# lslrh/DynaMask

Measured on AMD Instinct MI355X. Metric: img/s (DynaMask mask-head path, 512 RoIs/img, fixed 28x28 exit; ms_per_step = ms per RoI batch), higher is better.
Workload: dtype f32

## Files before the change

dynamask_amd/csrc/conv_igemm.hip:

```cpp
#include <type_traits>

#include "common.h"

namespace {

struct ConvArgs {
  const float* src[DM_MAX_SOURCES];
  int src_c[DM_MAX_SOURCES];
  long long src_bs[DM_MAX_SOURCES];
  int num_srcs;
  int NB, H, W, HW, Q;
  const float* wq;
  const float* bias;
  int KQ, Cout, CoutP;
  int relu;
  float* out;
  int out_ch_total, out_ch_offset;
  int Wp, plane;
  int MT;
  int q_begin = 0;
  int shuffle;
  const float* mask = nullptr;
  int off32 = 0;
  float* ws = nullptr;
// ... 2 lines not shown
  int want_split = 0;
  const float* addend = nullptr;
};

typedef __bf16 dm_bf16x8 __attribute__((ext_vector_type(8)));

__device__ __forceinline__ void dm_split3(float x, __bf16& h, __bf16& m, __bf16& l) {
  h = (__bf16)x;
  const float hf = (float)h;
  if (__builtin_isfinite(hf)) {
    const float r1 = x - hf;
    m = (__bf16)r1;
    l = (__bf16)(r1 - (float)m);
  } else {
    m = (__bf16)0.f;
    l = (__bf16)0.f;
  }
}

__device__ __forceinline__ void dm_split8x3(const dm_f32x4& q0, const dm_f32x4& q1, dm_f32x4 (&out)[3]) {
  dm_bf16x8 w[3];
#pragma unroll
  for (int e = 0; e < 8; ++e) {
    __bf16 h, m, l;
    dm_split3(e < 4 ? q0[e] : q1[e - 4], h, m, l);
    w[0][e] = h;
    w[1][e] = m;
    w[2][e] = l;
  }
#pragma unroll
  for (int p = 0; p < 3; ++p) out[p] = __builtin_bit_cast(dm_f32x4, w[p]);
}

template <int KS, int WGM, int WGN, int WM, int WN, int CK, int MAXPOS, int TAIL = 0, int PREC = 0, int POST = 0>
__device__ __forceinline__ void conv_igemm_body(const ConvArgs& a, const int bx, const int gx, const int by) {
  static_assert(TAIL == 0 || (TAIL == 4 && WGM == 1), "tail rows need a single cout tile");
  static_assert(PREC == 0 || (PREC == 1 && CK == 16 && TAIL == 0 && WM == 1 && WN == 2 && WGM == 2 && WGN == 2),
                "the bf16x3 build: 64 x 128 tiles, 16-channel chunks, no tail rows");
  static_assert(POST == 0 || (KS == 1 && TAIL == 0 && PREC == 0), "the post-activation addend: exact fp32 1x1 builds");
  constexpr int TM = WGM * WM * 32;
  constexpr int TMA = TM + TAIL;
  constexpr int TN = WGN * WN * 32;
  constexpr int NT = WGM * WGN * 64;
  constexpr int TAPS = KS * KS;
  constexpr int NQ = CK / 4;
  constexpr int NWC = PREC ? 6 : NQ;
  constexpr int A_F4 = TAPS * NWC * TMA;
  constexpr int A_PER_T = (A_F4 + NT - 1) / NT;
  constexpr int B1_PER_T = (NQ * TN + NT - 1) / NT;
  constexpr int BREG = (KS == 3) ? MAXPOS * NQ : B1_PER_T;

  extern __shared__ __attribute__((aligned(16))) float lds[];
  dm_f32x4* ldsA = reinterpret_cast<dm_f32x4*>(lds);
  dm_f32x4* ldsB = reinterpret_cast<dm_f32x4*>(lds) + A_F4;

  const int tid = threadIdx.x;
  const int lane = tid & 63;
  const int wave = tid >> 6;
  const int wave_m = wave / WGN;
  const int wave_n = wave % WGN;
  const int hi = lane >> 5;
  const int l31 = lane & 31;

  int m_tile, n_tile;
  {
    const int b = bx, grp = 8 * a.MT;
    const int full = (gx / grp) * grp;
    if (b < full) {
      const int g = b / grp, r = b - g * grp;
      m_tile = r / 8;
      n_tile = g * 8 + (r & 7);
    } else {
      const int r = b - full;
      m_tile = r % a.MT;
      n_tile = full / a.MT + r / a.MT;
    }
  }
  const int m0 = m_tile * TM;
  const int q0 = a.q_begin + n_tile * TN;
  const int HW = a.HW, W = a.W, H = a.H;
  const int plane = a.plane;
  int k_skip = 0, k_left = 0x7fffffff;
  float* e_out = a.out;
  const float* e_bias = a.bias;
  const float* e_mask = a.mask;
  int e_relu = a.relu, e_oct = a.out_ch_total, e_oco = a.out_ch_offset;
  if (a.ksplit > 1) {
// ... 179 lines not shown
    } else if (KS == 3) {
#pragma unroll
      for (int k = 0; k < MAXPOS; ++k) {
        const bool ok = st_n[k] >= 0;
        const float* gp = sp + b_off[k];
#pragma unroll
        for (int qd = 0; qd < NQ; ++qd) {
          dm_f32x4 v = {0.f, 0.f, 0.f, 0.f};
#pragma unroll
          for (int e = 0; e < 4; ++e) {
            const int ci = qd * 4 + e;
            if (ok && ci < ckv) v[e] = gp[(size_t)ci * HW];
          }
          rb[k * NQ + qd] = v;
        }
      }
    } else {
      const bool ok = st_n[0] >= 0;
      const float* gp = sp + b_off[0];
#pragma unroll
      for (int i = 0; i < B1_PER_T; ++i) {
        const int qd = PREC ? (tid / TN) * 2 + i : tid / TN + i * (NT / TN);
        dm_f32x4 v = {0.f, 0.f, 0.f, 0.f};
#pragma unroll
        for (int e = 0; e < 4; ++e) {
          const int ci = qd * 4 + e;
          if (ok && qd < NQ && ci < ckv) v[e] = gp[(size_t)ci * HW];
        }
        rb[i] = v;
      }
    }
  };

  auto commit = [&]() {
#pragma unroll
    for (int i = 0; i < A_PER_T; ++i) {
      const int idx = tid + i * NT;
      if (idx < A_F4) ldsA[idx] = ra[i];
    }
    if (PREC) {
      if (KS == 3) {
#pragma unroll
        for (int k = 0; k < MAXPOS; ++k) {
          const int pos = tid + k * NT;
          if (pos < plane) {
#pragma unroll
            for (int h8 = 0; h8 < 2; ++h8) {
              dm_f32x4 wd[3];
              dm_split8x3(rb[k * NQ + 2 * h8], rb[k * NQ + 2 * h8 + 1], wd);
#pragma unroll
              for (int p_ = 0; p_ < 3; ++p_) ldsB[(3 * h8 + p_) * plane + pos] = wd[p_];
            }
          }
        }
      } else {
        static_assert(!PREC || KS == 3 || (B1_PER_T == 2 && NT / TN == 2), "1x1 bf16x3 build: two quads (one half) per thread");
        const int h8 = tid / TN;
        dm_f32x4 wd[3];
        dm_split8x3(rb[0], rb[B1_PER_T > 1 ? 1 : 0], wd);
#pragma unroll
        for (int p_ = 0; p_ < 3; ++p_) ldsB[(3 * h8 + p_) * plane + (tid % TN)] = wd[p_];
      }
    } else if (KS == 3) {
#pragma unroll
      for (int k = 0; k < MAXPOS; ++k) {
        const int pos = tid + k * NT;
        if (pos < plane) {
#pragma unroll
          for (int qd = 0; qd < NQ; ++qd) ldsB[qd * plane + pos] = rb[k * NQ + qd];
        }
      }
    } else {
#pragma unroll
      for (int i = 0; i < B1_PER_T; ++i) {
        const int qd = tid / TN + i * (NT / TN);
        if (qd < NQ) ldsB[qd * plane + (tid % TN)] = rb[i];
      }
    }
  };

  for (; k_skip > 0 && cs < a.num_srcs; --k_skip) chunk_advance();
  if (chunk_valid()) prefetch();
  while (chunk_valid()) {
    const int ckv_cur = min(CK, curC - cc0);
    const int ngroups = (ckv_cur + 7) / 8;
    commit();
    __syncthreads();
    chunk_advance();
    --k_left;
    if (chunk_valid()) prefetch();

    if (PREC) {
      auto load_frag = [&](int tap, dm_f32x4 (*av)[3], dm_f32x4 (*bv)[3]) {
        const int tapoff = (KS == 3) ? ((tap / 3) * Wp + (tap % 3)) : 0;
#pragma unroll
        for (int i = 0; i < WM; ++i)
#pragma unroll
          for (int p_ = 0; p_ < 3; ++p_) av[i][p_] = ldsA[(tap * NWC + 3 * hi + p_) * TMA + (wave_m * WM + i) * 32 + l31];
#pragma unroll
        for (int j = 0; j < WN; ++j)
#pragma unroll
          for (int p_ = 0; p_ < 3; ++p_) bv[j][p_] = ldsB[p_ * plane + lane_base[j] + tapoff];
      };
      auto mfma = [&](const dm_f32x4& x, const dm_f32x4& y, dm_f32x16& c) {
        c = __builtin_amdgcn_mfma_f32_32x32x16_bf16(__builtin_bit_cast(dm_bf16x8, x), __builtin_bit_cast(dm_bf16x8, y), c, 0, 0, 0);
      };
      dm_f32x4 av[2][WM][3], bv[2][WN][3];
      load_frag(0, av[0], bv[0]);
#pragma unroll
      for (int st = 0; st < TAPS; ++st) {
        const int cur = st & 1;
        if (st + 1 < TAPS) load_frag(st + 1, av[cur ^ 1], bv[cur ^ 1]);
#pragma unroll
        for (int i = 0; i < WM; ++i)
#pragma unroll
          for (int j = 0; j < WN; ++j) {
            mfma(av[cur][i][2], bv[cur][j][0], accx[i][j]);
            mfma(av[cur][i][1], bv[cur][j][1], accx[i][j]);
            mfma(av[cur][i][0], bv[cur][j][2], accx[i][j]);
            mfma(av[cur][i][1], bv[cur][j][0], accx[i][j]);
            mfma(av[cur][i][0], bv[cur][j][1], accx[i][j]);
            mfma(av[cur][i][0], bv[cur][j][0], acc[i][j]);
          }
      }
    } else {
      constexpr int NG = NQ / 2;
      constexpr int STEPS = TAPS * NG;
      auto load_frag = [&](int st, dm_f32x4* av, dm_f32x4* bv) {
        const int tap = st / NG, g = st - tap * NG;
        const int tapoff = (KS == 3) ? ((tap / 3) * Wp + (tap % 3)) : 0;
#pragma unroll
        for (int i = 0; i < WM; ++i) av[i] = ldsA[(tap * NQ + 2 * g + hi) * TMA + (wave_m * WM + i) * 32 + l31];
        if (TAIL) av[WM] = ldsA[(tap * NQ + 2 * g + hi) * TMA + TM + (lane & 3)];
#pragma unroll
        for (int j = 0; j < WN; ++j) bv[j] = ldsB[(2 * g) * plane + lane_base[j] + tapoff];
      };
      dm_f32x4 av[2][WM + (TAIL ? 1 : 0)], bv[2][WN];
      load_frag(0, av[0], bv[0]);
#pragma unroll
      for (int st = 0; st < STEPS; ++st) {
        const int cur = st & 1;
        const bool live = (NG == 1) || ((st % NG) < ngroups);
        if (st + 1 < STEPS) load_frag(st + 1, av[cur ^ 1], bv[cur ^ 1]);
        if (live) {
#pragma unroll
          for (int e = 0; e < 4; ++e)
#pragma unroll
            for (int i = 0; i < WM; ++i)
#pragma unroll
              for (int j = 0; j < WN; ++j)
                acc[i][j] = __builtin_amdgcn_mfma_f32_32x32x2f32(av[cur][i][e], bv[cur][j][e], acc[i][j], 0, 0, 0);
          if (TAIL) {
#pragma unroll
            for (int e = 0; e < 4; ++e)
#pragma unroll
              for (int j = 0; j < WN; ++j)
                acct[j] = __builtin_amdgcn_mfma_f32_4x4x1f32(av[cur][WM][e], bv[cur][j][e], acct[j], 0, 0, 0);
          }
        }
      }
    }
    __syncthreads();
  }

  if (PREC) {
#pragma unroll
    for (int i = 0; i < WMX; ++i)
#pragma unroll
      for (int j = 0; j < WNX; ++j)
#pragma unroll
        for (int r = 0; r < 16; ++r) acc[i][j][r] += accx[i][j][r];
  }

  if (a.shuffle == 0) {
    float* pj[WN];
#pragma unroll
    for (int j = 0; j < WN; ++j)
      pj[j] = e_out + ((size_t)col_n[j] * e_oct + e_oco) * HW + col_p[j];
    const int co_lane = m0 + wave_m * WM * 32 + 4 * hi;
    const size_t off_lane = (size_t)co_lane * HW;
    const bool relu = e_relu & 1;
    float bias_r[WM][16];
#pragma unroll
    for (int i = 0; i < WM; ++i)
#pragma unroll
      for (int r = 0; r < 16; ++r) bias_r[i][r] = 0.f;
    if (e_bias) {
#pragma unroll
      for (int i = 0; i < WM; ++i)
#pragma unroll
        for (int r = 0; r < 16; ++r) bias_r[i][r] = e_bias[min(co_lane + i * 32 + (r & 3) + 8 * (r >> 2), a.Cout - 1)];
#pragma unroll
      for (int i = 0; i < WM; ++i)
#pragma unroll
        for (int r = 0; r < 16; ++r) asm volatile("" : "+v"(bias_r[i][r]));
// ... 61 lines not shown
          const float b = e_bias ? e_bias[oc] : 0.f;
#pragma unroll
          for (int j = 0; j < WN; ++j) {
            if (col_ok[j]) {
              float v = acc[i][j][r] + b;
              if (e_relu & 1) v = fmaxf(v, 0.f);
              e_out[(((size_t)col_n[j] * a.shuffle + oc) * (2 * H) + 2 * sy[j] + dy) * (2 * W) + 2 * sx[j] + dx] = v;
            }
          }
        }
      }
    }
  }
  if (TAIL) {
#pragma unroll
    for (int j = 0; j < WN; ++j) {
#pragma unroll
      for (int i = 0; i < 4; ++i) {
        float v = acct[j][i] + __shfl_xor(acct[j][i], 32, 64);
        const int co = m0 + TM + i;
        if (hi == 0 && co < a.Cout && col_ok[j]) {
          if (e_bias) v += e_bias[co];
          float* op = e_out + ((size_t)col_n[j] * e_oct + e_oco + co) * HW + col_p[j];
          if (e_relu & 2) v += *op;
          if (e_relu & 1) v = fmaxf(v, 0.f);
          if (e_mask && !(e_mask[op - e_out] > 0.f)) v = 0.f;
          *op = v;
        }
      }
    }
  }
}

template <int KS, int WGM, int WGN, int WM, int WN, int CK, int MAXPOS, int TAIL = 0, int PREC = 0, int POST = 0>
__global__ __launch_bounds__(WGM* WGN * 64, PREC ? (KS == 1 ? 3 : 2) : (KS == 3 && WGM == 2 && WGN == 2 && WM == 2 && WN == 2 && MAXPOS == 1) || (KS == 1 && CK == 16) ? 3 : 1) void conv_igemm_kernel(ConvArgs a) {
  conv_igemm_body<KS, WGM, WGN, WM, WN, CK, MAXPOS, TAIL, PREC, POST>(a, (int)blockIdx.x, (int)gridDim.x, (int)blockIdx.y);
}

struct ConvGroup {
  ConvArgs a[3];
  int end[3];
};
template <int KS, int WGM, int WGN, int WM, int WN, int CK, int MAXPOS, int PREC = 0>
__global__ __launch_bounds__(WGM* WGN * 64, (KS == 1 && CK == 16 && WM == 1) ? 3 : (WGM == 2 && WGN == 2 && WM == 2 && WN == 2) ? 2 : 1) void conv_igemm_group_kernel(ConvGroup g) {
  const int b = (int)blockIdx.x, by = (int)blockIdx.y;
  if (b < g.end[0]) conv_igemm_body<KS, WGM, WGN, WM, WN, CK, MAXPOS, 0, PREC>(g.a[0], b, g.end[0], by);
  else if (b < g.end[1]) conv_igemm_body<KS, WGM, WGN, WM, WN, CK, MAXPOS, 0, PREC>(g.a[1], b - g.end[0], g.end[1] - g.end[0], by);
  else conv_igemm_body<KS, WGM, WGN, WM, WN, CK, MAXPOS, 0, PREC>(g.a[2], b - g.end[1], g.end[2] - g.end[1], by);
}

struct PackArgs {
  const float* w;
  float* wq;
  int Cout, Cin, kk, flip;
  int rows, cols, colsP;
  int nsrc;
  int src_c[DM_MAX_SOURCES];
  int KQ;
  int deconv;
};

__device__ __forceinline__ void pack_weight_body(const PackArgs& p, int ld, int c0) {
  const long long total = (long long)p.kk * p.KQ * p.colsP * 4;
  for (long long idx = (long long)blockIdx.x * blockDim.x + threadIdx.x; idx < total;
       idx += (long long)gridDim.x * blockDim.x) {
    const int e = (int)(idx & 3);
    const int col = (int)((idx >> 2) % p.colsP);
    const int kq = (int)((idx >> 2) / p.colsP % p.KQ);
    const int tap = (int)((idx >> 2) / ((long long)p.colsP * p.KQ));
    int pc = kq * 4 + e, row = -1, base = 0;
    for (int s = 0; s < p.nsrc; ++s) {
      const int padded = (p.src_c[s] + 7) / 8 * 8;
      if (pc < padded) {
        if (pc < p.src_c[s]) row = base + pc;
        break;
      }
      pc -= padded;
      base += p.src_c[s];
    }
    float v = 0.f;
    if (row >= 0 && col < p.cols) {
// ... 143 lines not shown
  splitk_reduce_body<V4>(ws, splits, stride, NB, Cout, HW, bias, flags, out, out_ch_total, out_ch_offset, mask);
}

struct ReduceGroup {
  const float* ws[3];
  const float* bias[3];
  float* out[3];
};
template <bool V4>
__global__ __launch_bounds__(256) void conv_splitk_reduce_group_kernel(ReduceGroup r, int splits, long long stride, int NB,
                                                                      int Cout, int HW, int flags) {
  const int p = (int)blockIdx.y;
  splitk_reduce_body<V4>(r.ws[p], splits, stride, NB, Cout, HW, r.bias[p], flags, r.out[p], Cout, 0, nullptr);
}

static int conv_split_choice(int chunks, bool k3, int Smax, long long out_floats) {
  const double chain_us = chunks * (k3 ? 2.1 : 1.5), out_mb = (double)out_floats * 4e-6;
  double best = 8.0;
  int S = 1;
  for (int c = 2; c <= Smax; ++c) {
    const double g = chain_us * (1.0 - 1.0 / c) - (5.0 + (c + 1) * out_mb * 0.25);
    if (g > best) { best = g; S = c; }
  }
  return S;
}

template <int KS, int WGM, int WGN, int WM, int WN, int CK, int MAXPOS, int TAIL = 0, int PREC = 0, int POST = 0>
int launch_conv_mp(ConvArgs& a, hipStream_t st) {
  constexpr int TM = WGM * WM * 32;
  constexpr int TN = WGN * WN * 32;
  constexpr int NT = WGM * WGN * 64;
  const int NTiles = dm_ceil_div(a.Q - a.q_begin, TN);
  constexpr int NWC = PREC ? 6 : CK / 4;
  const size_t lds_bytes = 16 * ((size_t)KS * KS * NWC * (TM + TAIL) + (size_t)NWC * a.plane);
  if (lds_bytes > 64 * 1024) {
    if (!PREC || lds_bytes > 80 * 1024) return DM_ERR_UNSUPPORTED;
    static bool raised[DM_MAX_DEVICES] = {false};
    const int rc = dm_ensure_lds_limit(reinterpret_cast<const void*>(&conv_igemm_kernel<KS, WGM, WGN, WM, WN, CK, MAXPOS, TAIL, PREC, POST>),
                                       80 * 1024, raised);
    if (rc != DM_OK) return rc;
  }
  a.ksplit = 1;
  if (a.ws && a.shuffle == 0 && a.q_begin == 0 && !POST) {
    constexpr int CKS = CK;
    int chunks = 0;
    for (int s_ = 0; s_ < a.num_srcs; ++s_) chunks += dm_ceil_div(a.src_c[s_], CKS);
    const int wgs = a.MT * NTiles, cus = dm_num_cus();
    const long long per = (long long)a.NB * a.Cout * a.HW;
    int Smax = a.want_split > 0 ? min(a.want_split, chunks / 4) : min(min(8, (3 * cus) / max(wgs, 1)), chunks / 4);
    if (per > 0) Smax = (int)min((long long)Smax, a.ws_floats / per);
    const int S = conv_split_choice(chunks, KS == 3, Smax, per);
    if (S >= 2) {
      a.kchunks = dm_ceil_div(chunks, S);
      a.ksplit = dm_ceil_div(chunks, a.kchunks);
      a.ws_stride = per;
    }
  }
  if (a.ksplit > 1) {
    const float* bias = a.bias;
    const float* mask = a.mask;
    float* out = a.out;
    const int flags = a.relu, oct = a.out_ch_total, oco = a.out_ch_offset;
    DM_LAUNCH((conv_igemm_kernel<KS, WGM, WGN, WM, WN, CK, MAXPOS, TAIL, PREC, POST>), dim3(a.MT * NTiles, a.ksplit), dim3(NT), lds_bytes, st, a);
    int rc = dm_check_launch();
    if (rc != DM_OK) return rc;
    const long long total = a.ws_stride;
    const bool v4 = (a.HW & 3) == 0 && (total & 3) == 0 && total < 0x7fffffffLL &&
                    ((((uintptr_t)a.ws) | ((uintptr_t)out) | ((uintptr_t)mask)) & 15) == 0;
    if (v4)
      DM_LAUNCH(conv_splitk_reduce_kernel<true>, dim3((unsigned)min((long long)4096, (total / 4 + 255) / 256)), dim3(256), 0, st, a.ws,
                a.ksplit, a.ws_stride, a.NB, a.Cout, a.HW, bias, flags, out, oct, oco, mask);
    else
      DM_LAUNCH(conv_splitk_reduce_kernel<false>, dim3((unsigned)min((long long)4096, (total + 255) / 256)), dim3(256), 0, st, a.ws,
                a.ksplit, a.ws_stride, a.NB, a.Cout, a.HW, bias, flags, out, oct, oco, mask);
    return dm_check_launch();
  }
  DM_LAUNCH((conv_igemm_kernel<KS, WGM, WGN, WM, WN, CK, MAXPOS, TAIL, PREC, POST>), dim3(a.MT * NTiles), dim3(NT), lds_bytes, st, a);
  return dm_check_launch();
}

template <int KS, int WGM, int WGN, int WM, int WN, int CK, int TAIL = 0, int PREC = 0, int POST = 0>
int launch_conv(ConvArgs& a, hipStream_t st) {
  constexpr int TM = WGM * WM * 32;
  constexpr int TN = WGN * WN * 32;
  constexpr int NT = WGM * WGN * 64;
  a.MT = TAIL ? 1 : dm_ceil_div(a.CoutP, TM);
  if (KS == 3) {
    a.Wp = a.W + 2;
    const int nsegmax = dm_ceil_div(TN - 1, a.HW) + 1;
    const int rmax = dm_ceil_div(TN - 1, a.W) + 1 + 2 * nsegmax;
    a.plane = rmax * a.Wp;
    if constexpr (PREC != 0) {
      if (a.plane <= NT) return launch_conv_mp<KS, WGM, WGN, WM, WN, CK, 1, TAIL, PREC>(a, st);
      return DM_ERR_UNSUPPORTED;
    } else {
      if (a.plane <= NT) return launch_conv_mp<KS, WGM, WGN, WM, WN, CK, 1, TAIL>(a, st);
      if (a.plane <= 2 * NT) return launch_conv_mp<KS, WGM, WGN, WM, WN, CK, 2, TAIL>(a, st);
      if (a.plane <= 4 * NT) return launch_conv_mp<KS, WGM, WGN, WM, WN, CK, 4, TAIL>(a, st);
      return DM_ERR_UNSUPPORTED;
    }
  }
  a.Wp = 0;
  a.plane = TN;
  return launch_conv_mp<KS, WGM, WGN, WM, WN, CK, 1, TAIL, PREC, POST>(a, st);
}

template <int KS, int WGM, int WGN, int WM, int WN, int CK, int MAXPOS>
int launch_group_mp(ConvGroup& g, int count, int S, float* ws, hipStream_t st) {
  constexpr int TN = WGN * WN * 32;
  constexpr int TM = WGM * WM * 32;
  const ConvArgs& a0 = g.a[0];
  const size_t lds_bytes = 16 * ((size_t)KS * KS * (CK / 4) * TM + (size_t)(CK / 4) * a0.plane);
  if (lds_bytes > 64 * 1024) return DM_ERR_UNSUPPORTED;
  int chunks = dm_ceil_div(a0.src_c[0], CK);
  const long long per = (long long)a0.NB * a0.Cout * a0.HW;
  int total = 0;
  for (int i = 0; i < 3; ++i) {
    ConvArgs& a = g.a[i];
    a.ksplit = 1;
    if (S >= 2) {
      a.kchunks = dm_ceil_div(chunks, S);
      a.ksplit = dm_ceil_div(chunks, a.kchunks);
      a.ws = ws + (size_t)min(i, count - 1) * S * per;
      a.ws_stride = per;
      a.ws_floats = (long long)S * per;
    }
    if (i < count) total += a.MT * dm_ceil_div(a.Q, TN);
    g.end[i] = total;
  }
  const int splits = g.a[0].ksplit;
  DM_LAUNCH((conv_igemm_group_kernel<KS, WGM, WGN, WM, WN, CK, MAXPOS>), dim3((unsigned)total, (unsigned)splits), dim3(WGM * WGN * 64),
            lds_bytes, st, g);
  int rc = dm_check_launch();
  if (rc != DM_OK || splits < 2) return rc;
  ReduceGroup r;
  for (int i = 0; i < 3; ++i) {
    const ConvArgs& a = g.a[min(i, count - 1)];
    r.ws[i] = a.ws; r.bias[i] = a.bias; r.out[i] = a.out;
  }
  bool v4 = (a0.HW & 3) == 0 && (per & 3) == 0 && per < 0x7fffffffLL && (((uintptr_t)ws) & 15) == 0 && (S * per & 3) == 0;
  for (int i = 0; i < count; ++i) v4 = v4 && (((uintptr_t)g.a[i].out) & 15) == 0;
  const int flags = a0.relu & 1;
  if (v4)
    DM_LAUNCH(conv_splitk_reduce_group_kernel<true>, dim3((unsigned)min((long long)4096, (per / 4 + 255) / 256), (unsigned)count),
              dim3(256), 0, st, r, splits, per, a0.NB, a0.Cout, a0.HW, flags);
  else
    DM_LAUNCH(conv_splitk_reduce_group_kernel<false>, dim3((unsigned)min((long long)4096, (per + 255) / 256), (unsigned)count),
              dim3(256), 0, st, r, splits, per, a0.NB, a0.Cout, a0.HW, flags);
  return dm_check_launch();
}

template <int KS, int WGM, int WGN, int WM, int WN, int CK>
int launch_group(ConvGroup& g, int count, int S, float* ws, hipStream_t st) {
  constexpr int TM = WGM * WM * 32;
  constexpr int TN = WGN * WN * 32;
  constexpr int NT = WGM * WGN * 64;
  for (int i = 0; i < 3; ++i) {
    ConvArgs& a = g.a[i];
    a.MT = dm_ceil_div(a.CoutP, TM);
    if (KS == 3) {
      a.Wp = a.W + 2;
      const int nsegmax = dm_ceil_div(TN - 1, a.HW) + 1;
      a.plane = (dm_ceil_div(TN - 1, a.W) + 1 + 2 * nsegmax) * a.Wp;
    } else {
      a.Wp = 0;
// ... 20 lines not shown
  long long wgs, slots;
  if (Cout > 64) {
    slots = 2LL * cus;
    wgs = (long long)count * dm_ceil_div((Cout + 31) / 32 * 32, 128) * dm_ceil_div(Q, 128);
    if (wgs >= slots) return 1;
  } else {
    slots = 3LL * cus;
    wgs = (long long)count * dm_ceil_div(Q, 128);
  }
  long long Smax = min(8LL, slots / max(wgs, 1LL));
  Smax = min(Smax, ws_floats / ((long long)count * per));
  Smax = min(Smax, (long long)(chunks / 4));
  if (Smax < 2) return 1;
  return conv_split_choice(chunks, true, (int)Smax, per);
}

int run_pack_bf16x3(PackArgs& p, hipStream_t st) {
  const long long total = (long long)p.kk * (p.KQ / 3) * p.colsP;
  const int blocks = (int)min((long long)dm_ceil_div(total, 256), 4096LL);
  DM_LAUNCH(pack_weight_bf16x3_kernel, dim3(blocks), dim3(256), 0, st, p);
  return dm_check_launch();
}

int run_pack(PackArgs& p, hipStream_t st) {
  const long long total = (long long)p.kk * p.KQ * p.colsP * 4;
  const int blocks = (int)min((long long)dm_ceil_div(total, 256), 4096LL);
  DM_LAUNCH(pack_weight_kernel, dim3(blocks), dim3(256), 0, st, p);
  return dm_check_launch();
}

}

extern "C" int dm_conv_packed_cout(int Cout) { return (Cout + 31) / 32 * 32; }

extern "C" long long dm_conv_packed_floats(int Cout, int ksize, int num_srcs, const int* src_channels) {
  if (Cout <= 0 || ksize <= 0 || num_srcs < 1 || num_srcs > DM_MAX_SOURCES || !src_channels) return -1;
  return (long long)ksize * ksize * packed_quads(num_srcs, src_channels) * dm_conv_packed_cout(Cout) * 4;
}

extern "C" int dm_conv_pack_weight(const float* w_oihw, int Cout, int Cin, int ksize, int transpose_flip,
                                   int num_srcs, const int* src_channels, float* w_packed, dm_stream_t stream) {
  if (!w_oihw || !w_packed || Cout <= 0 || Cin <= 0 || (ksize != 1 && ksize != 3)) return DM_ERR_INVALID_ARG;
  if (num_srcs < 1 || num_srcs > DM_MAX_SOURCES || !src_channels) return DM_ERR_INVALID_ARG;
  PackArgs p;
  p.w = w_oihw; p.wq = w_packed; p.Cout = Cout; p.Cin = Cin; p.kk = ksize * ksize; p.flip = transpose_flip ? 1 : 0;
  p.rows = transpose_flip ? Cout : Cin;
  p.cols = transpose_flip ? Cin : Cout;
  p.colsP = dm_conv_packed_cout(p.cols);
  p.nsrc = num_srcs;
  int sum = 0;
  for (int s = 0; s < DM_MAX_SOURCES; ++s) {
    p.src_c[s] = s < num_srcs ? src_channels[s] : 0;
    if (s < num_srcs && src_channels[s] <= 0) return DM_ERR_INVALID_ARG;
    sum += p.src_c[s];
  }
  if (sum != p.rows) return DM_ERR_INVALID_ARG;
  p.KQ = packed_quads(num_srcs, src_channels);
  p.deconv = 0;
  return run_pack(p, (hipStream_t)stream);
}

extern "C" long long dm_conv_packed_floats_bf16x3(int Cout, int ksize, int num_srcs, const int* src_channels) {
  if (Cout <= 0 || ksize <= 0 || num_srcs < 1 || num_srcs > DM_MAX_SOURCES || !src_channels) return -1;
  return (long long)ksize * ksize * packed_words_bf16x3(num_srcs, src_channels) * dm_conv_packed_cout(Cout) * 4;
}

// ... 225 lines not shown
  if (bf16x3) return launch_conv<1, 2, 2, 1, 2, 16, 0, 1>(a, (hipStream_t)stream);
  return launch_conv<1, 2, 2, 2, 2, 16>(a, (hipStream_t)stream);
}

extern "C" int dm_conv1x1_group_fwd(int count, const float* const* x, const int* Cin, const int* H, const int* W, int NB,
                                    const float* const* w_packed, const float* const* bias, const int* Cout, int relu,
                                    float* const* out, dm_stream_t stream) {
  if (count < 1 || count > 3 || !x || !Cin || !H || !W || !w_packed || !bias || !Cout || !out || NB < 0) return DM_ERR_INVALID_ARG;
  if (relu & ~17) return DM_ERR_INVALID_ARG;
  const bool bf16x3 = (relu & 16) != 0;
  if (NB == 0) return DM_OK;
  ConvGroup g;
  int total = 0;
  constexpr int TM = 64, TN = 128;
  for (int i = 0; i < 3; ++i) {
    const int j = i < count ? i : count - 1;
    if (!x[j] || !w_packed[j] || !out[j] || Cin[j] <= 0 || H[j] <= 0 || W[j] <= 0 || Cout[j] <= 0) return DM_ERR_INVALID_ARG;
    if ((long long)NB * H[j] * W[j] > 0x7fffffffLL) return DM_ERR_INVALID_ARG;
    ConvArgs& a = g.a[i];
    for (int s = 0; s < DM_MAX_SOURCES; ++s) { a.src[s] = nullptr; a.src_c[s] = 0; a.src_bs[s] = 0; }
    a.src[0] = x[j]; a.src_c[0] = Cin[j]; a.src_bs[0] = (long long)Cin[j] * H[j] * W[j]; a.num_srcs = 1;
    a.KQ = bf16x3 ? packed_words_bf16x3(1, a.src_c) : packed_quads(1, a.src_c);
    a.NB = NB; a.H = H[j]; a.W = W[j]; a.HW = H[j] * W[j]; a.Q = NB * H[j] * W[j];
    a.wq = w_packed[j]; a.bias = bias[j]; a.Cout = Cout[j]; a.CoutP = dm_conv_packed_cout(Cout[j]);
    a.relu = relu & 1; a.out = out[j]; a.out_ch_total = Cout[j]; a.out_ch_offset = 0;
    a.shuffle = 0; a.q_begin = 0; a.mask = nullptr; a.ws = nullptr; a.ksplit = 1;
    a.off32 = ((long long)NB * a.src_bs[0] * 4 < (1LL << 32)) ? 1 : 0;
    a.MT = dm_ceil_div(a.CoutP, TM);
    a.Wp = 0; a.plane = TN;
    if (i < count) total += a.MT * dm_ceil_div(a.Q, TN);
    g.end[i] = total;
  }
  const size_t nwc = bf16x3 ? 6 : 16 / 4;
  const size_t lds_bytes = 16 * (nwc * TM + nwc * TN);
  if (bf16x3)
    DM_LAUNCH((conv_igemm_group_kernel<1, 2, 2, 1, 2, 16, 1, 1>), dim3((unsigned)total), dim3(256), lds_bytes, (hipStream_t)stream, g);
  else
    DM_LAUNCH((conv_igemm_group_kernel<1, 2, 2, 1, 2, 16, 1>), dim3((unsigned)total), dim3(256), lds_bytes, (hipStream_t)stream, g);
  return dm_check_launch();
}

static int conv2d_group_setup(int count, const float* const* x, int NB, int H, int W, int Cin, int Cout, int ksize,
                              const float* const* w_packed, const float* const* bias, int relu, float* const* out, int shuffle,
                              ConvGroup& g) {
  if (count < 1 || count > 3 || !x || !w_packed || !out || NB < 0 || H <= 0 || W <= 0 || Cin <= 0 || Cout <= 0)
    return DM_ERR_INVALID_ARG;
  if ((long long)NB * H * W > 0x7fffffffLL) return DM_ERR_INVALID_ARG;
  if (relu & ~(1 | 8 | 16)) return DM_ERR_INVALID_ARG;
  if (relu & 16) return DM_ERR_UNSUPPORTED;
  for (int i = 0; i < count && NB > 0; ++i)
    if (!x[i] || !w_packed[i] || !out[i]) return DM_ERR_INVALID_ARG;
  const int couts = shuffle ? 4 * Cout : Cout;
  for (int i = 0; i < 3; ++i) {
    const int j = i < count ? i : count - 1;
    ConvArgs& a = g.a[i];
    for (int s = 0; s < DM_MAX_SOURCES; ++s) { a.src[s] = nullptr; a.src_c[s] = 0; a.src_bs[s] = 0; }
    a.src[0] = x[j]; a.src_c[0] = Cin; a.src_bs[0] = (long long)Cin * H * W; a.num_srcs = 1;
    a.KQ = packed_quads(1, a.src_c);
    a.NB = NB; a.H = H; a.W = W; a.HW = H * W; a.Q = NB * H * W;
    a.wq = w_packed[j]; a.bias = bias ? bias[j] : nullptr; a.Cout = couts; a.CoutP = dm_conv_packed_cout(couts);
    a.relu = relu & 1;
    if (!shuffle && (long long)NB * Cout * H * W * 4 > (192LL << 20)) a.relu |= 4;
    a.out = out[j]; a.out_ch_total = shuffle ? 0 : Cout; a.out_ch_offset = 0;
    a.shuffle = shuffle; a.q_begin = 0; a.mask = nullptr; a.ws = nullptr; a.ws_floats = 0; a.ws_stride = 0;
    a.ksplit = 1; a.kchunks = 0; a.want_split = 0;
    a.off32 = ((long long)NB * a.src_bs[0] * 4 < (1LL << 32)) ? 1 : 0;
  }
  return DM_OK;
}

extern "C" int dm_conv2d_group_splits(int count, int NB, int H, int W, int Cin, int Cout, int ksize, long long workspace_floats) {
// ... 49 lines not shown
```

dynamask_amd/ops.py:

```python
import ctypes

import torch

from . import _abi, hazard
from . import precision as _precision
from ._lib import check, lib


import os

WEIGHT_EPOCH = [0]

DETERMINISTIC = [os.environ.get('DM_DETERMINISTIC', '0') == '1']


def _fx_like(t):
    return torch.zeros(t.shape, device=t.device, dtype=torch.int64)


def _fx_finish(fx, out, accumulate):
    check(lib().dm_fx_to_float(_p(fx), fx.numel(), _p(out), 1 if accumulate else 0, 0, _stream()), 'dm_fx_to_float')
    return out


# ... 678 lines not shown
    for s in srcs:
        assert s.shape[0] == NB and s.shape[2] == H and s.shape[3] == W
    cin = sum(s.shape[1] for s in srcs)
    layout = conv_layout(w_packed)
    assert w_packed.numel() == packed_floats(cout, ksize, [s.shape[1] for s in srcs], layout), 'weights packed for other sources'
    if out is None:
        out = torch.empty((NB, cout, H, W), device=srcs[0].device, dtype=torch.float32)
    else:
        _chk(out, 'out')
        assert out.shape[0] == NB and out.shape[2] == H and out.shape[3] == W
    strides = (ctypes.c_longlong * len(srcs))(*[int(s.stride(0)) for s in srcs])
    flags = (1 if relu else 0) | (2 if accumulate else 0) | (8 if _overlapped else 0) | (16 if layout == 'bf16x3' else 0)
    if mask is not None:
        _chk(mask, 'mask')
        assert mask.shape == out.shape
        rc = lib().dm_conv2d_fwd_masked(_ptr_array(srcs), _int_array([s.shape[1] for s in srcs]), strides, len(srcs), NB, H, W,
                                        _p(w_packed), _p(bias), cout, ksize, flags, _p(out), out.shape[1], out_ch_offset,
                                        _p(mask), _stream())
        check(rc, 'dm_conv2d_fwd_masked')
        return out
    if CONV_SPLITK[0] and _SPLITK_DEPTH[0] > 0 and not accumulate:
        nws = int(lib().dm_conv2d_splitk_floats(NB, H, W, cout, ksize))
        if nws > 0:
            ws = torch.empty((nws,), device=out.device, dtype=torch.float32)
            rc = lib().dm_conv2d_fwd_ws(_ptr_array(srcs), _int_array([s.shape[1] for s in srcs]), strides, len(srcs), NB, H, W,
                                        _p(w_packed), _p(bias), cout, ksize, flags, _p(out), out.shape[1], out_ch_offset,
                                        _p(ws), nws, _stream())
            check(rc, 'dm_conv2d_fwd_ws')
            return out
    rc = lib().dm_conv2d_fwd(_ptr_array(srcs), _int_array([s.shape[1] for s in srcs]), strides, len(srcs), NB, H, W,
                             _p(w_packed), _p(bias), cout, ksize, flags, _p(out), out.shape[1], out_ch_offset, _stream())
    check(rc, 'dm_conv2d_fwd')
    return out


def conv1x1_group(xs, w_packeds, biases, couts, relu=False, outs=None):
    k = len(xs)
    assert 1 <= k <= 3 and len(w_packeds) == k and len(biases) == k and len(couts) == k
    NB = xs[0].shape[0]
    for x, w in zip(xs, w_packeds):
        _chk(x, 'x')
        _chk(w, 'w_packed')
        assert x.shape[0] == NB
    layout = conv_layout(w_packeds[0])
    assert all(conv_layout(w) == layout for w in w_packeds), 'weights of one group packed in different layouts'
    for x, w, c in zip(xs, w_packeds, couts):
        assert w.numel() == packed_floats(c, 1, [x.shape[1]], layout), 'weights packed for other sources'
    if outs is None:
        outs = [torch.empty((NB, c, x.shape[2], x.shape[3]), device=x.device, dtype=torch.float32) for x, c in zip(xs, couts)]
    for o, x, c in zip(outs, xs, couts):
        _chk(o, 'out')
        assert tuple(o.shape) == (NB, c, x.shape[2], x.shape[3])
    bias_arr = (ctypes.c_void_p * k)(*[0 if b is None else _chk(b, 'bias').data_ptr() for b in biases])
    if hazard.ENABLED[0]:
        hazard.note_ptr_array(bias_arr, [b for b in biases if b is not None])
    check(lib().dm_conv1x1_group_fwd(k, _ptr_array(xs), _int_array([x.shape[1] for x in xs]), _int_array([x.shape[2] for x in xs]),
                                     _int_array([x.shape[3] for x in xs]), NB, _ptr_array(w_packeds), bias_arr, _int_array(couts),
                                     (1 if relu else 0) | (16 if layout == 'bf16x3' else 0), _ptr_array(outs), _stream()),
          'dm_conv1x1_group_fwd')
    return outs


def deform_conv(x, offset, w_packed, cout, deform_groups, relu=False, out=None):
    _chk(x, 'x')
    _chk(offset, 'offset')
    _chk(w_packed, 'w_packed')
# ... 1515 lines not shown
```

include/dynamask_hip.h:

```cpp
#ifndef DYNAMASK_HIP_H
#define DYNAMASK_HIP_H

#include <stdint.h>

#ifdef __cplusplus
extern "C" {
#endif

#define DM_OK 0
#define DM_ERR_INVALID_ARG (-1)
#define DM_ERR_LAUNCH (-2)
#define DM_ERR_UNSUPPORTED (-3)

#define DM_MAX_LEVELS 4
#define DM_MAX_SOURCES 4

typedef void* dm_stream_t;

const char* dm_error_string(int code);
#define DM_ABI_VERSION 28
int dm_abi_version(void);
const char* dm_build_info(void);
int dm_reload_env_knobs(void);

// ... 8 lines not shown
                        long long workspace_bytes, dm_stream_t stream);

int dm_roi_align_bwd(const float* grad_out, float* const* grad_feats, const int* H, const int* W,
                     const float* spatial_scales, int num_levels, int B, int C, const float* rois, int N,
                     int P, int sampling_ratio, float finest_scale, dm_stream_t stream);

int dm_conv_packed_cout(int Cout);
long long dm_conv_packed_floats(int Cout, int ksize, int num_srcs, const int* src_channels);
int dm_conv_pack_weight(const float* w_oihw, int Cout, int Cin, int ksize, int transpose_flip,
                        int num_srcs, const int* src_channels, float* w_packed, dm_stream_t stream);

typedef struct dm_pack_job {
  const float* w;
  float* w_packed;
  int Cout, Cin, ksize, transpose_flip;
  int num_srcs, src_channels[DM_MAX_SOURCES];
  int ld, c0;
} dm_pack_job;
int dm_conv_pack_weight_batch(const dm_pack_job* jobs_device, int num_jobs, dm_stream_t stream);

long long dm_conv_packed_floats_bf16x3(int Cout, int ksize, int num_srcs, const int* src_channels);
int dm_conv_pack_weight_bf16x3(const float* w_oihw, int Cout, int Cin, int ksize, int transpose_flip,
                               int num_srcs, const int* src_channels, float* w_packed, dm_stream_t stream);

int dm_conv2d_fwd(const float* const* srcs, const int* src_channels, const long long* src_batch_strides,
                  int num_srcs, int NB, int H, int W,
                  const float* w_packed, const float* bias, int Cout, int ksize, int relu, float* out,
                  int out_ch_total, int out_ch_offset, dm_stream_t stream);
long long dm_conv2d_splitk_floats(int NB, int H, int W, int Cout, int ksize);
int dm_conv2d_fwd_ws(const float* const* srcs, const int* src_channels, const long long* src_batch_strides,
                     int num_srcs, int NB, int H, int W, const float* w_packed, const float* bias, int Cout, int ksize,
                     int relu, float* out, int out_ch_total, int out_ch_offset, float* workspace,
                     long long workspace_floats, dm_stream_t stream);

int dm_conv1x1_group_fwd(int count, const float* const* x, const int* Cin, const int* H, const int* W, int NB,
                         const float* const* w_packed, const float* const* bias, const int* Cout, int relu, float* const* out,
                         dm_stream_t stream);

int dm_conv2d_fwd_masked(const float* const* srcs, const int* src_channels, const long long* src_batch_strides,
                         int num_srcs, int NB, int H, int W, const float* w_packed, const float* bias, int Cout,
                         int ksize, int relu, float* out, int out_ch_total, int out_ch_offset, const float* mask,
                         dm_stream_t stream);

int dm_point_sample_fwd(const float* feat, int B, int C, int H, int W, const float* rois, int N, int S,
                        float spatial_scale, float* out, dm_stream_t stream);

int dm_class_logits_fwd(const float* x, int N, int C, int HW, const float* w_inst, const float* b_inst,
                        const float* w_det, const float* b_det, int num_classes, const int64_t* labels,
                        float* inst, float* det, float* sig_out, int sig_ch_total, int sig_ch_offset,
                        dm_stream_t stream);

int dm_stage_head_fwd(const float* sem, int B, int Cs, int H, int W, const float* rois, int N, int S, float spatial_scale,
                      float* sampled, const float* x, int C, const float* w_inst, const float* b_inst, const float* w_det,
                      const float* b_det, int num_classes, const int64_t* labels, float* inst, float* det, float* sig_out,
                      int sig_ch_total, int sig_ch_offset, dm_stream_t stream);

int dm_class_logits_up2x_fwd(const float* x, int N, int C, int H, int W, const float* w_inst, const float* b_inst,
                             const float* w_det, const float* b_det, int num_classes, const int64_t* labels,
                             float* inst, float* det, dm_stream_t stream);

int dm_deform_conv_fwd(const float* x, const float* offset, int NB, int C, int H, int W,
                       const float* w_packed, int Cout, int deform_groups, int relu, float* out,
                       dm_stream_t stream);
int dm_deform_conv_tout_supported(int NB, int C, int H, int W, int Cout, int M2);
int dm_deform_conv_tout_fwd(const float* x, const float* offset, int NB, int C, int H, int W, const float* w_packed, int Cout,
                            int deform_groups, const float* w2t, const float* b2, int M2, float* out2, int out2_ch_total,
// ... 289 lines not shown
```

Baseline: 287.2.

## Double-buffer conv LDS tiles to drop the trailing barrier per chunk

Adds a PIPE build of the implicit-GEMM conv kernel that allocates two LDS images and alternates chunks between them. This removes the second __syncthreads per K chunk, so the commit of the next chunk can overlap with other waves still reading the previous one. It applies to selected 1x1 and 3x3 tile configurations when doubled LDS fits in 64 KB, and a runtime toggle is exported. The doubled LDS footprint can lower occupancy, since launch bounds request 3 blocks per CU for some builds.

After: 286.9. About the same (-0.1%).

```diff
diff --git a/dynamask_amd/csrc/conv_igemm.hip b/dynamask_amd/csrc/conv_igemm.hip
--- a/dynamask_amd/csrc/conv_igemm.hip
+++ b/dynamask_amd/csrc/conv_igemm.hip
@@ -58,8 +58,16 @@
   for (int p = 0; p < 3; ++p) out[p] = __builtin_bit_cast(dm_f32x4, w[p]);
 }
 
-template <int KS, int WGM, int WGN, int WM, int WN, int CK, int MAXPOS, int TAIL = 0, int PREC = 0, int POST = 0>
+constexpr bool conv_pipe_build(int KS, int WGM, int WGN, int WM, int WN, int CK, int PREC) {
+  return !PREC && ((KS == 1 && CK == 16 && WGM == 2 && WGN == 2 && WN == 2 && (WM == 1 || WM == 2)) ||
+                   (KS == 3 && CK == 8 && WGM == 1 && WGN == 4 && WM == 1 && WN == 1));
+}
+static int g_conv_pipe = 1;
+
+template <int KS, int WGM, int WGN, int WM, int WN, int CK, int MAXPOS, int TAIL = 0, int PREC = 0, int POST = 0, int PIPE = 0>
 __device__ __forceinline__ void conv_igemm_body(const ConvArgs& a, const int bx, const int gx, const int by) {
+  static_assert(PIPE == 0 || (PIPE == 1 && conv_pipe_build(KS, WGM, WGN, WM, WN, CK, PREC)),
+                "one barrier per chunk: the 16-channel 1x1 builds at 128 / 64 x 128 and the 3x3 32-cout x 128-pixel builds");
   static_assert(TAIL == 0 || (TAIL == 4 && WGM == 1), "tail rows need a single cout tile");
   static_assert(PREC == 0 || (PREC == 1 && CK == 16 && TAIL == 0 && WM == 1 && WN == 2 && WGM == 2 && WGN == 2),
                 "the bf16x3 build: 64 x 128 tiles, 16-channel chunks, no tail rows");
@@ -77,8 +85,8 @@
   constexpr int BREG = (KS == 3) ? MAXPOS * NQ : B1_PER_T;
 
   extern __shared__ __attribute__((aligned(16))) float lds[];
-  dm_f32x4* ldsA = reinterpret_cast<dm_f32x4*>(lds);
-  dm_f32x4* ldsB = reinterpret_cast<dm_f32x4*>(lds) + A_F4;
+  dm_f32x4* const ldsA = reinterpret_cast<dm_f32x4*>(lds);
+  dm_f32x4* const ldsB = reinterpret_cast<dm_f32x4*>(lds) + A_F4;
 
   const int tid = threadIdx.x;
   const int lane = tid & 63;
@@ -324,11 +332,11 @@
     }
   };
 
-  auto commit = [&]() {
+  auto commit = [&](dm_f32x4* const cA, dm_f32x4* const cB) {
 #pragma unroll
     for (int i = 0; i < A_PER_T; ++i) {
       const int idx = tid + i * NT;
-      if (idx < A_F4) ldsA[idx] = ra[i];
+      if (idx < A_F4) cA[idx] = ra[i];
     }
     if (PREC) {
       if (KS == 3) {
@@ -341,7 +349,7 @@
               dm_f32x4 wd[3];
               dm_split8x3(rb[k * NQ + 2 * h8], rb[k * NQ + 2 * h8 + 1], wd);
 #pragma unroll
-              for (int p_ = 0; p_ < 3; ++p_) ldsB[(3 * h8 + p_) * plane + pos] = wd[p_];
+              for (int p_ = 0; p_ < 3; ++p_) cB[(3 * h8 + p_) * plane + pos] = wd[p_];
             }
           }
         }
@@ -351,7 +359,7 @@
         dm_f32x4 wd[3];
         dm_split8x3(rb[0], rb[B1_PER_T > 1 ? 1 : 0], wd);
 #pragma unroll
-        for (int p_ = 0; p_ < 3; ++p_) ldsB[(3 * h8 + p_) * plane + (tid % TN)] = wd[p_];
+        for (int p_ = 0; p_ < 3; ++p_) cB[(3 * h8 + p_) * plane + (tid % TN)] = wd[p_];
       }
     } else if (KS == 3) {
 #pragma unroll
@@ -359,24 +367,33 @@
         const int pos = tid + k * NT;
         if (pos < plane) {
 #pragma unroll
-          for (int qd = 0; qd < NQ; ++qd) ldsB[qd * plane + pos] = rb[k * NQ + qd];
+          for (int qd = 0; qd < NQ; ++qd) cB[qd * plane + pos] = rb[k * NQ + qd];
         }
       }
     } else {
 #pragma unroll
       for (int i = 0; i < B1_PER_T; ++i) {
         const int qd = tid / TN + i * (NT / TN);
-        if (qd < NQ) ldsB[qd * plane + (tid % TN)] = rb[i];
+        if (qd < NQ) cB[qd * plane + (tid % TN)] = rb[i];
       }
     }
   };
 
   for (; k_skip > 0 && cs < a.num_srcs; --k_skip) chunk_advance();
   if (chunk_valid()) prefetch();
+  constexpr int UNR = (PIPE && KS == 1) ? 2 : 1;
+  const int img_slots = A_F4 + NWC * (KS == 1 ? TN : plane);
+  int img_var = 0;
   while (chunk_valid()) {
+#pragma unroll
+    for (int img = 0; img < UNR; ++img) {
+    if (img == 1 && !chunk_valid()) break;
+    const int ioff = (KS == 1) ? img * img_slots : img_var;
+    dm_f32x4* const cA = ldsA + ioff;
+    dm_f32x4* const cB = ldsB + ioff;
     const int ckv_cur = min(CK, curC - cc0);
     const int ngroups = (ckv_cur + 7) / 8;
-    commit();
+    commit(cA, cB);
     __syncthreads();
     chunk_advance();
     --k_left;
@@ -388,11 +405,11 @@
 #pragma unroll
         for (int i = 0; i < WM; ++i)
 #pragma unroll
-          for (int p_ = 0; p_ < 3; ++p_) av[i][p_] = ldsA[(tap * NWC + 3 * hi + p_) * TMA + (wave_m * WM + i) * 32 + l31];
+          for (int p_ = 0; p_ < 3; ++p_) av[i][p_] = cA[(tap * NWC + 3 * hi + p_) * TMA + (wave_m * WM + i) * 32 + l31];
 #pragma unroll
         for (int j = 0; j < WN; ++j)
 #pragma unroll
-          for (int p_ = 0; p_ < 3; ++p_) bv[j][p_] = ldsB[p_ * plane + lane_base[j] + tapoff];
+          for (int p_ = 0; p_ < 3; ++p_) bv[j][p_] = cB[p_ * plane + lane_base[j] + tapoff];
       };
       auto mfma = [&](const dm_f32x4& x, const dm_f32x4& y, dm_f32x16& c) {
         c = __builtin_amdgcn_mfma_f32_32x32x16_bf16(__builtin_bit_cast(dm_bf16x8, x), __builtin_bit_cast(dm_bf16x8, y), c, 0, 0, 0);
@@ -422,10 +439,10 @@
         const int tap = st / NG, g = st - tap * NG;
         const int tapoff = (KS == 3) ? ((tap / 3) * Wp + (tap % 3)) : 0;
 #pragma unroll
-        for (int i = 0; i < WM; ++i) av[i] = ldsA[(tap * NQ + 2 * g + hi) * TMA + (wave_m * WM + i) * 32 + l31];
-        if (TAIL) av[WM] = ldsA[(tap * NQ + 2 * g + hi) * TMA + TM + (lane & 3)];
-#pragma unroll
-        for (int j = 0; j < WN; ++j) bv[j] = ldsB[(2 * g) * plane + lane_base[j] + tapoff];
+        for (int i = 0; i < WM; ++i) av[i] = cA[(tap * NQ + 2 * g + hi) * TMA + (wave_m * WM + i) * 32 + l31];
+        if (TAIL) av[WM] = cA[(tap * NQ + 2 * g + hi) * TMA + TM + (lane & 3)];
+#pragma unroll
+        for (int j = 0; j < WN; ++j) bv[j] = cB[(2 * g) * plane + lane_base[j] + tapoff];
       };
       dm_f32x4 av[2][WM + (TAIL ? 1 : 0)], bv[2][WN];
       load_frag(0, av[0], bv[0]);
@@ -452,7 +469,9 @@
         }
       }
     }
-    __syncthreads();
+    if (!PIPE) __syncthreads();
+    if (PIPE && KS == 3) img_var = img_slots - img_var;
+    }
   }
 
   if (PREC) {
@@ -580,21 +599,21 @@
   }
 }
 
-template <int KS, int WGM, int WGN, int WM, int WN, int CK, int MAXPOS, int TAIL = 0, int PREC = 0, int POST = 0>
+template <int KS, int WGM, int WGN, int WM, int WN, int CK, int MAXPOS, int TAIL = 0, int PREC = 0, int POST = 0, int PIPE = 0>
 __global__ __launch_bounds__(WGM* WGN * 64, PREC ? (KS == 1 ? 3 : 2) : (KS == 3 && WGM == 2 && WGN == 2 && WM == 2 && WN == 2 && MAXPOS == 1) || (KS == 1 && CK == 16) ? 3 : 1) void conv_igemm_kernel(ConvArgs a) {
-  conv_igemm_body<KS, WGM, WGN, WM, WN, CK, MAXPOS, TAIL, PREC, POST>(a, (int)blockIdx.x, (int)gridDim.x, (int)blockIdx.y);
+  conv_igemm_body<KS, WGM, WGN, WM, WN, CK, MAXPOS, TAIL, PREC, POST, PIPE>(a, (int)blockIdx.x, (int)gridDim.x, (int)blockIdx.y);
 }
 
 struct ConvGroup {
   ConvArgs a[3];
   int end[3];
 };
-template <int KS, int WGM, int WGN, int WM, int WN, int CK, int MAXPOS, int PREC = 0>
+template <int KS, int WGM, int WGN, int WM, int WN, int CK, int MAXPOS, int PREC = 0, int PIPE = 0>
 __global__ __launch_bounds__(WGM* WGN * 64, (KS == 1 && CK == 16 && WM == 1) ? 3 : (WGM == 2 && WGN == 2 && WM == 2 && WN == 2) ? 2 : 1) void conv_igemm_group_kernel(ConvGroup g) {
   const int b = (int)blockIdx.x, by = (int)blockIdx.y;
-  if (b < g.end[0]) conv_igemm_body<KS, WGM, WGN, WM, WN, CK, MAXPOS, 0, PREC>(g.a[0], b, g.end[0], by);
-  else if (b < g.end[1]) conv_igemm_body<KS, WGM, WGN, WM, WN, CK, MAXPOS, 0, PREC>(g.a[1], b - g.end[0], g.end[1] - g.end[0], by);
-  else conv_igemm_body<KS, WGM, WGN, WM, WN, CK, MAXPOS, 0, PREC>(g.a[2], b - g.end[1], g.end[2] - g.end[1], by);
+  if (b < g.end[0]) conv_igemm_body<KS, WGM, WGN, WM, WN, CK, MAXPOS, 0, PREC, 0, PIPE>(g.a[0], b, g.end[0], by);
+  else if (b < g.end[1]) conv_igemm_body<KS, WGM, WGN, WM, WN, CK, MAXPOS, 0, PREC, 0, PIPE>(g.a[1], b - g.end[0], g.end[1] - g.end[0], by);
+  else conv_igemm_body<KS, WGM, WGN, WM, WN, CK, MAXPOS, 0, PREC, 0, PIPE>(g.a[2], b - g.end[1], g.end[2] - g.end[1], by);
 }
 
 struct PackArgs {
@@ -804,7 +823,10 @@
   constexpr int NT = WGM * WGN * 64;
   const int NTiles = dm_ceil_div(a.Q - a.q_begin, TN);
   constexpr int NWC = PREC ? 6 : CK / 4;
-  const size_t lds_bytes = 16 * ((size_t)KS * KS * NWC * (TM + TAIL) + (size_t)NWC * a.plane);
+  const size_t img_bytes = 16 * ((size_t)KS * KS * NWC * (TM + TAIL) + (size_t)NWC * a.plane);
+  constexpr bool PIPE_BUILD = conv_pipe_build(KS, WGM, WGN, WM, WN, CK, PREC);
+  const bool pipe = PIPE_BUILD && g_conv_pipe && 2 * img_bytes <= 64 * 1024;
+  const size_t lds_bytes = pipe ? 2 * img_bytes : img_bytes;
   if (lds_bytes > 64 * 1024) {
     if (!PREC || lds_bytes > 80 * 1024) return DM_ERR_UNSUPPORTED;
     static bool raised[DM_MAX_DEVICES] = {false};
@@ -833,7 +855,10 @@
     const float* mask = a.mask;
     float* out = a.out;
     const int flags = a.relu, oct = a.out_ch_total, oco = a.out_ch_offset;
-    DM_LAUNCH((conv_igemm_kernel<KS, WGM, WGN, WM, WN, CK, MAXPOS, TAIL, PREC, POST>), dim3(a.MT * NTiles, a.ksplit), dim3(NT), lds_bytes, st, a);
+    if constexpr (PIPE_BUILD) {
+      if (pipe) DM_LAUNCH((conv_igemm_kernel<KS, WGM, WGN, WM, WN, CK, MAXPOS, TAIL, PREC, POST, 1>), dim3(a.MT * NTiles, a.ksplit), dim3(NT), lds_bytes, st, a);
+    }
+    if (!pipe) DM_LAUNCH((conv_igemm_kernel<KS, WGM, WGN, WM, WN, CK, MAXPOS, TAIL, PREC, POST>), dim3(a.MT * NTiles, a.ksplit), dim3(NT), lds_bytes, st, a);
     int rc = dm_check_launch();
     if (rc != DM_OK) return rc;
     const long long total = a.ws_stride;
@@ -847,7 +872,10 @@
                 a.ksplit, a.ws_stride, a.NB, a.Cout, a.HW, bias, flags, out, oct, oco, mask);
     return dm_check_launch();
   }
-  DM_LAUNCH((conv_igemm_kernel<KS, WGM, WGN, WM, WN, CK, MAXPOS, TAIL, PREC, POST>), dim3(a.MT * NTiles), dim3(NT), lds_bytes, st, a);
+  if constexpr (PIPE_BUILD) {
+    if (pipe) DM_LAUNCH((conv_igemm_kernel<KS, WGM, WGN, WM, WN, CK, MAXPOS, TAIL, PREC, POST, 1>), dim3(a.MT * NTiles), dim3(NT), lds_bytes, st, a);
+  }
+  if (!pipe) DM_LAUNCH((conv_igemm_kernel<KS, WGM, WGN, WM, WN, CK, MAXPOS, TAIL, PREC, POST>), dim3(a.MT * NTiles), dim3(NT), lds_bytes, st, a);
   return dm_check_launch();
 }
 
@@ -882,7 +910,10 @@
   constexpr int TN = WGN * WN * 32;
   constexpr int TM = WGM * WM * 32;
   const ConvArgs& a0 = g.a[0];
-  const size_t lds_bytes = 16 * ((size_t)KS * KS * (CK / 4) * TM + (size_t)(CK / 4) * a0.plane);
+  const size_t img_bytes = 16 * ((size_t)KS * KS * (CK / 4) * TM + (size_t)(CK / 4) * a0.plane);
+  constexpr bool PIPE_BUILD = conv_pipe_build(KS, WGM, WGN, WM, WN, CK, 0);
+  const bool pipe = PIPE_BUILD && g_conv_pipe && 2 * img_bytes <= 64 * 1024;
+  const size_t lds_bytes = pipe ? 2 * img_bytes : img_bytes;
   if (lds_bytes > 64 * 1024) return DM_ERR_UNSUPPORTED;
   int chunks = dm_ceil_div(a0.src_c[0], CK);
   const long long per = (long long)a0.NB * a0.Cout * a0.HW;
@@ -901,8 +932,12 @@
     g.end[i] = total;
   }
   const int splits = g.a[0].ksplit;
-  DM_LAUNCH((conv_igemm_group_kernel<KS, WGM, WGN, WM, WN, CK, MAXPOS>), dim3((unsigned)total, (unsigned)splits), dim3(WGM * WGN * 64),
-            lds_bytes, st, g);
+  if constexpr (PIPE_BUILD) {
+    if (pipe) DM_LAUNCH((conv_igemm_group_kernel<KS, WGM, WGN, WM, WN, CK, MAXPOS, 0, 1>), dim3((unsigned)total, (unsigned)splits),
+                        dim3(WGM * WGN * 64), lds_bytes, st, g);
+  }
+  if (!pipe) DM_LAUNCH((conv_igemm_group_kernel<KS, WGM, WGN, WM, WN, CK, MAXPOS>), dim3((unsigned)total, (unsigned)splits), dim3(WGM * WGN * 64),
+                       lds_bytes, st, g);
   int rc = dm_check_launch();
   if (rc != DM_OK || splits < 2) return rc;
   ReduceGroup r;
@@ -989,6 +1024,12 @@
 }
 
 extern "C" int dm_conv_packed_cout(int Cout) { return (Cout + 31) / 32 * 32; }
+
+extern "C" int dm_conv_pipeline(int mode) {
+  const int was = g_conv_pipe;
+  if (mode >= 0) g_conv_pipe = mode ? 1 : 0;
+  return was;
+}
 
 extern "C" long long dm_conv_packed_floats(int Cout, int ksize, int num_srcs, const int* src_channels) {
   if (Cout <= 0 || ksize <= 0 || num_srcs < 1 || num_srcs > DM_MAX_SOURCES || !src_channels) return -1;
@@ -1280,11 +1321,13 @@
     g.end[i] = total;
   }
   const size_t nwc = bf16x3 ? 6 : 16 / 4;
-  const size_t lds_bytes = 16 * (nwc * TM + nwc * TN);
+  const size_t img_bytes = 16 * (nwc * TM + nwc * TN);
   if (bf16x3)
-    DM_LAUNCH((conv_igemm_group_kernel<1, 2, 2, 1, 2, 16, 1, 1>), dim3((unsigned)total), dim3(256), lds_bytes, (hipStream_t)stream, g);
+    DM_LAUNCH((conv_igemm_group_kernel<1, 2, 2, 1, 2, 16, 1, 1>), dim3((unsigned)total), dim3(256), img_bytes, (hipStream_t)stream, g);
+  else if (g_conv_pipe)
+    DM_LAUNCH((conv_igemm_group_kernel<1, 2, 2, 1, 2, 16, 1, 0, 1>), dim3((unsigned)total), dim3(256), 2 * img_bytes, (hipStream_t)stream, g);
   else
-    DM_LAUNCH((conv_igemm_group_kernel<1, 2, 2, 1, 2, 16, 1>), dim3((unsigned)total), dim3(256), lds_bytes, (hipStream_t)stream, g);
+    DM_LAUNCH((conv_igemm_group_kernel<1, 2, 2, 1, 2, 16, 1>), dim3((unsigned)total), dim3(256), img_bytes, (hipStream_t)stream, g);
   return dm_check_launch();
 }
 
diff --git a/dynamask_amd/ops.py b/dynamask_amd/ops.py
--- a/dynamask_amd/ops.py
+++ b/dynamask_amd/ops.py
@@ -734,6 +734,10 @@
                              _p(w_packed), _p(bias), cout, ksize, flags, _p(out), out.shape[1], out_ch_offset, _stream())
     check(rc, 'dm_conv2d_fwd')
     return out
+
+
+def conv_pipeline(mode=-1):
+    return int(lib().dm_conv_pipeline(int(mode)))
 
 
 def conv1x1_group(xs, w_packeds, biases, couts, relu=False, outs=None):
diff --git a/include/dynamask_hip.h b/include/dynamask_hip.h
--- a/include/dynamask_hip.h
+++ b/include/dynamask_hip.h
@@ -64,6 +64,8 @@
                      int num_srcs, int NB, int H, int W, const float* w_packed, const float* bias, int Cout, int ksize,
                      int relu, float* out, int out_ch_total, int out_ch_offset, float* workspace,
                      long long workspace_floats, dm_stream_t stream);
+
+int dm_conv_pipeline(int mode);
 
 int dm_conv1x1_group_fwd(int count, const float* const* x, const int* Cin, const int* H, const int* W, int NB,
                          const float* const* w_packed, const float* const* bias, const int* Cout, int relu, float* const* out,
```
